# thu-nics/Rad-NeRF

Measured on AMD Instinct MI355X. Metric: million samples/s fwd+bwd, 8192 rays, model_zoo_size=2; rgb L∞ vs ref, higher is better.
Workload: dtype f16/f32

## Files before the change

### include/radnerf.h

```cpp
#ifndef RADNERF_H
#define RADNERF_H

#include <stdint.h>

#ifdef __cplusplus
extern "C" {
#endif

#define RN_ABI_VERSION 9
#define RN_FX_STATS_BYTES 640
int rn_version(void);
const char* rn_last_error(void);
const char* rn_abi_signatures(void);
void rn_set_debug_flags(int flags);
int rn_debug_cycles(unsigned long long* out);
int rn_set_level_pairing(uint64_t pairing);

int rn_ray_aabb_intersect(const float* rays_o, const float* rays_d, const float* centers,
                          const float* half_sizes, int64_t n_rays, int64_t n_voxels,
                          int32_t max_hits, int32_t* hit_cnt, float* hits_t,
                          int64_t* hits_voxel_idx, void* stream);

int rn_ray_sphere_intersect(const float* rays_o, const float* rays_d, const float* centers,
                            const float* radii, int64_t n_rays, int64_t n_spheres,
// ... 182 lines not shown
int rn_igrad_to_f32(int64_t n, int32_t* igrad_lo, int32_t* igrad_carry, const float* scale,
                    float* grid_grad, void* stream);

int rn_field_fwd_merged(const float* ts, const int32_t* ray_of, const float* rays_o,
                        const float* rays_d, const int32_t* seg_base, const int32_t* seg_count,
                        const int32_t* chunk_desc, int32_t* queue,
                        int64_t n_rays, int32_t n_models, const void* grid_f16,
                        const uint32_t* level_offset, const uint32_t* level_hsize,
                        const uint32_t* level_res, const float* level_scale,
                        const float* xyz_min, const float* extent, const void* frags,
                        float* sigma, float* rgb, void* feat_cache, const int32_t* mstart,
                        const int32_t* perm, int32_t blocks, int32_t threads, void* stream);

int rn_field_fwd_levels(const float* ts, const int32_t* ray_of, const float* rays_o,
                        const float* rays_d, const int32_t* seg_base, const int32_t* seg_count,
                        int64_t n_rays, int32_t n_models, const void* grid_f16,
                        const uint32_t* level_offset, const uint32_t* level_hsize,
                        const uint32_t* level_res, const float* level_scale,
                        const float* xyz_min, const float* extent, const void* frags,
                        float* sigma, float* rgb, void* feat_cache, const int32_t* mstart,
                        const int32_t* perm, uint32_t* planes, int64_t plane_stride, void* prep,
                        int32_t prep_ready, int32_t enc_blocks, int32_t mlp_blocks, int32_t* xq,
                        void* stream);

int rn_gate_fwd(const float* in0, const float* in1, int32_t stride, int64_t n_rays,
                int32_t n_models, const void* frags, float* gate, float* importance,
                int32_t n_blocks, void* stream);
int rn_gate_bwd(const float* in0, const float* in1, int32_t stride, int64_t n_rays,
                int32_t n_models, const void* frags, const float* dL_dgate, float* dw,
                int32_t n_params, const void* dinput_frags, float* dL_dinput,
                int32_t n_blocks, void* stream);

int rn_field_dinput(const float* xyzs, const float* dirs, int64_t n_samples, const float* ts,
                    const int32_t* ray_of, const float* rays_o, const float* rays_d,
                    const int32_t* seg_base, const int32_t* seg_count, int32_t n_models,
                    const void* grid_f16, const uint32_t* level_offset,
                    const uint32_t* level_hsize, const uint32_t* level_res,
                    const float* level_scale, const float* xyz_min, const float* extent,
                    const void* frags, const void* dinput_frags, const float* dL_dsigma,
                    const float* dL_drgb, const void* feat_cache, float* dL_dxyz,
                    float* dL_ddir, int32_t blocks_per_model, void* stream);
int rn_density_update_sampled(const void* grid_ptrs, const void* bitfield_ptrs, int32_t n_models,
                              int32_t cascades, int32_t grid_size, float scale,
                              float density_threshold, float decay, uint64_t seed,
                              const void* grid_f16, const uint32_t* level_offset,
                              const uint32_t* level_hsize, const uint32_t* level_res,
// ... 90 lines not shown
```

### rad-nerf_amd/csrc/field.hip

```cpp
#include "rn_field.h"
#include "rn_bin.h"
#pragma clang fp contract(off)

static int g_field_dbg = 0;
static uint64_t g_level_pairing = 0;
__device__ unsigned long long g_rn_cyc[8];

namespace {

template <int MODE, int CACHE>
__global__ void __launch_bounds__(256, FWD_MIN_WAVES)
k_field_fwd(FieldArgs a) {
    __shared__ __attribute__((aligned(16))) rn_half sW[FIELD_FWD_FRAGS * RN_FRAG_HALFS];
    __shared__ LvTab sT;
    const int k = blockIdx.y;
    rn_block_copy16(sW, a.frags + (size_t)k * FIELD_FRAGS * RN_FRAG_HALFS,
                    FIELD_FWD_FRAGS * RN_FRAG_BYTES);
    lv_stage(sT, a.gm);
    __syncthreads();
    int64_t base, n;
    sample_range(a, MODE, k, base, n);
    const int64_t n_tiles = (n + 31) / 32;
    const int waves = blockDim.x / RN_WAVE;
    const int lane = rn_lane(), h = lane >> 5;
    for (int64_t tile = (int64_t)blockIdx.x * waves + threadIdx.x / RN_WAVE; tile < n_tiles;
         tile += (int64_t)gridDim.x * waves) {
        rn_lds_order();
        FwdState st;
// ... 1123 lines not shown
    }
    lv_stage(sT, a.gm);
    const int waves = blockDim.x / RN_WAVE;
    const int wid = __builtin_amdgcn_readfirstlane(threadIdx.x / RN_WAVE);
    const int lane = rn_lane(), c = lane & 31, h = lane >> 5;
    int ticket = 0, n_chunks = 0;
    if (threadIdx.x == 0) { n_chunks = m.queue[1]; ticket = atomicAdd(m.queue + 2, 1); }

    auto mlp_tile = [&](const int32_t* ch, int u) {
        const int k = u % K, t = u / K;
        const int n_k = ch[2 + FM_KMAX + k];
        if (t * 32 >= n_k) return;
        rn_lds_order();
        const int i = t * 32 + c;
        const bool valid = i < n_k;
        const int64_t s = ch[2 + k] + (valid ? i : 0);
        FwdState st;
        float ux, uy, uz;
        constexpr int TC = ENC_M ? CACHE_READ_NT : CACHE;
        const rn_half* W = GW ? a.frags + (size_t)k * FIELD_FRAGS * RN_FRAG_HALFS
                              : sWm + (size_t)k * FIELD_FWD_FRAGS * RN_FRAG_HALFS;
        tile_forward_s<1, TC>(a, sT, W, s, valid, TC != CACHE_NONE ? cache_slot(a, s) : nullptr,
                              st, ux, uy, uz);
        if (valid && h == 0) {
            a.sigma[s] = expf(st.g0);
            a.rgb[3 * s + 0] = sigmoidf(st.out[0]);
            a.rgb[3 * s + 1] = sigmoidf(st.out[1]);
            a.rgb[3 * s + 2] = sigmoidf(st.out[2]);
        }
    };
    auto mlp_tiles = [&](const int32_t* ch) {
        int max_t = 0;
        for (int k = 0; k < K; ++k) max_t = max(max_t, (ch[2 + FM_KMAX + k] + 31) >> 5);
        return max_t * K;
    };

    bool prev_live = false;
    for (int it = 0;; ++it) {
        int32_t* cur = sCh[it & 1];
        const int32_t* prev = sCh[(it & 1) ^ 1];
        __syncthreads();
        if (threadIdx.x == 0) {
            const int ch = ticket;
            ticket = atomicAdd(m.queue + 2, 1);
            int4 d[CH_DESC / 4];
            if (ch < n_chunks) {
#pragma unroll
                for (int q = 0; q < CH_DESC / 4; ++q)
                    d[q] = reinterpret_cast<const int4*>(m.desc + (size_t)ch * CH_DESC)[q];
            }
            const int32_t* di = reinterpret_cast<const int32_t*>(d);
            cur[0] = ch < n_chunks ? di[0] : B;
// ... 14 lines not shown
        if (!live && !prev_live) break;
        int p_base = 0, n_p = 0;
        if (live) { p_base = m.mstart[cur[0]]; n_p = m.mstart[cur[1]] - p_base; }
        const int nA = (n_p + 31) >> 5;
        const int nB = prev_live ? mlp_tiles(prev) : 0;
        for (int u = wid; u < nA + nB; u += waves) {
            if (u >= nA) { mlp_tile(prev, u - nA); continue; }
            const int q = u * 32 + c;
            const bool valid = q < n_p;
            const int64_t s = m.perm[p_base + (valid ? q : 0)];
            float x, y, z, dx, dy, dz;
            load_sample<1>(a, s, x, y, z, dx, dy, dz);
            const float ux = unit_coord(x, a.xyz_min[0], a.extent[0]);
            const float uy = unit_coord(y, a.xyz_min[1], a.extent[1]);
            const float uz = unit_coord(z, a.xyz_min[2], a.extent[2]);
            half8 e0, e1;
            encode_lane(a, sT, rn_rsrc(a.grid, a.grid_bytes), h, ux, uy, uz, valid, e0, e1);
            if (valid) { half8* fc = cache_slot(a, s); fc[0] = e0; fc[1] = e1; }
        }
        prev_live = live;
    }
}


__global__ void __launch_bounds__(256)
k_enc_prep(FieldArgs a, MergeArgs m, float4* __restrict__ prep) {
    const int P = m.mstart[m.n_rays];
    for (int p = blockIdx.x * blockDim.x + threadIdx.x; p < P; p += gridDim.x * blockDim.x) {
        const int s = m.perm[p];
        float x, y, z, dx, dy, dz;
        load_sample<1>(a, s, x, y, z, dx, dy, dz);
        prep[p] = make_float4(unit_coord(x, a.xyz_min[0], a.extent[0]),
                              unit_coord(y, a.xyz_min[1], a.extent[1]),
                              unit_coord(z, a.xyz_min[2], a.extent[2]), __int_as_float(s));
    }
}

__global__ void __launch_bounds__(256)
k_field_encode_levels(FieldArgs a, MergeArgs m, const float4* __restrict__ prep,
                      int32_t* __restrict__ xq, uint64_t pairing) {
    __shared__ LvTab sT;
    lv_stage(sT, a.gm);
    __syncthreads();
    const int g = blockIdx.x & 7;
    if (xq && threadIdx.x == 0) {
        uint32_t xcc;
// ... 61 lines not shown
    for (int kb = k_lo; kb <= k_hi; kb += FM_LDS_K) {
        const int ke = min(k_hi, kb + FM_LDS_K - 1);
        __syncthreads();
        for (int k = kb; k <= ke; ++k)
            rn_block_copy16(sWm + (size_t)(k - kb) * FIELD_FWD_FRAGS * RN_FRAG_HALFS,
                            a.frags + (size_t)k * FIELD_FRAGS * RN_FRAG_HALFS,
                            FIELD_FWD_FRAGS * RN_FRAG_BYTES);
        __syncthreads();
        const int ua = max(u0, first[kb]), ub = min(u1, first[ke + 1]);
        for (int u = ua + wid; u < ub; u += waves) {
            int k = kb;
            while (k < ke && u >= first[k + 1]) ++k;
            const int t = u - first[k];
            const int n_k = sSeg[1][k];
            const int i = t * 32 + c;
            const bool valid = i < n_k;
            const int64_t s = sSeg[0][k] + (valid ? i : 0);
            FwdState st;
            float ux, uy, uz;
            rn_lds_order();
            tile_forward_s<1, CACHE_PLANES>(a, sT, sWm + (size_t)(k - kb) * FIELD_FWD_FRAGS * RN_FRAG_HALFS,
                                            s, valid, a.feat ? cache_slot(a, s) : nullptr, st,
                                            ux, uy, uz);
            if (valid && h == 0) {
                a.sigma[s] = expf(st.g0);
                a.rgb[3 * s + 0] = sigmoidf(st.out[0]);
                a.rgb[3 * s + 1] = sigmoidf(st.out[1]);
                a.rgb[3 * s + 2] = sigmoidf(st.out[2]);
            }
        }
    }
}


__global__ void __launch_bounds__(256)
k_seed_max(const int32_t* __restrict__ seg_base, const int32_t* __restrict__ seg_count,
           const float* __restrict__ sigma, const float* __restrict__ dsigma,
           const float* __restrict__ drgb, uint32_t* __restrict__ mbits) {
    const int k = blockIdx.y;
    const int64_t base = seg_base[k], n = seg_count[k];
    float mx = 0.f;
    for (int64_t i = (int64_t)blockIdx.x * blockDim.x + threadIdx.x; i < n;
         i += (int64_t)gridDim.x * blockDim.x) {
        const int64_t s = base + i;
        mx = fmaxf(mx, fabsf(dsigma[s] * sigma[s]));
        mx = fmaxf(mx, fmaxf(fabsf(drgb[3 * s]), fmaxf(fabsf(drgb[3 * s + 1]), fabsf(drgb[3 * s + 2]))));
    }
    mx = rn_wave_max(mx);
    if (rn_lane() == 0 && mx > 0.f && isfinite(mx)) atomicMax(mbits, __float_as_uint(mx));
}

__global__ void k_seed_scale(const uint32_t* __restrict__ mbits, float* __restrict__ scale) {
// ... 788 lines not shown
            RN_CHECK_LAUNCH();
            return 0;
        }
    }
    if (fx_mode == 5) {
        k_field_bwd_merged<CACHE_READ, false, 5><<<blocks, blk, 0, st>>>(a, m, G, F);
    } else if (fx_mode == 4) {
        k_field_bwd_merged<CACHE_READ, false, 4><<<blocks, blk, 0, st>>>(a, m, G, F);
    } else if (fx_mode == 2) {
        k_field_bwd_merged<CACHE_READ, false, 2><<<blocks, blk, 0, st>>>(a, m, G, F);
    } else if (fx_mode == 3) {
        k_field_bwd_merged<CACHE_READ, false, 3><<<blocks, blk, 0, st>>>(a, m, G, F);
    } else if (igrad_lo) {
        if (feat_cache) k_field_bwd_merged<CACHE_READ, false, 1><<<blocks, blk, 0, st>>>(a, m, G, F);
        else k_field_bwd_merged<CACHE_NONE, false, 1><<<blocks, blk, 0, st>>>(a, m, G, F);
    } else {
        if (feat_cache) k_field_bwd_merged<CACHE_READ, false, 0><<<blocks, blk, 0, st>>>(a, m, G, F);
        else k_field_bwd_merged<CACHE_NONE, false, 0><<<blocks, blk, 0, st>>>(a, m, G, F);
    }
    RN_CHECK_LAUNCH();
    return 0;
}

int rn_field_fwd_merged(const float* ts, const int32_t* ray_of, const float* rays_o,
                        const float* rays_d, const int32_t* seg_base, const int32_t* seg_count,
                        const int32_t* chunk_desc, int32_t* queue,
                        int64_t n_rays, int32_t n_models, const void* grid_f16,
                        const uint32_t* level_offset, const uint32_t* level_hsize,
                        const uint32_t* level_res, const float* level_scale,
                        const float* xyz_min, const float* extent, const void* frags,
                        float* sigma, float* rgb, void* feat_cache, const int32_t* mstart,
                        const int32_t* perm, int32_t blocks, int32_t threads, void* stream) {
    RN_CHECK_ARG(n_rays >= 1 && n_models >= 1 && n_models <= FM_KMAX && blocks >= 1,
                 "bad sizes (n_models <= 8)");
    RN_CHECK_ARG(threads >= 64 && threads <= 1024 && threads % 64 == 0, "threads: 64..1024, waves");
    RN_CHECK_ARG(ts && ray_of && rays_o && rays_d && seg_base && seg_count &&
                 chunk_desc && queue && grid_f16 && level_offset && level_hsize && level_res &&
                 level_scale && xyz_min && extent && frags && sigma && rgb, "null pointer");
    RN_CHECK_ARG(!(mstart || perm) || (mstart && perm && feat_cache),
                 "merged-order encoding needs mstart, perm and the encoding cache");
    FieldArgs a{};
    fill_args(a, xyz_min, extent, level_offset, level_hsize, level_res, level_scale);
    a.dbg = rn_dbg(g_field_dbg);
    a.grid = (const rn_half*)grid_f16; a.frags = (const rn_half*)frags;
    a.sigma = sigma; a.rgb = rgb; a.feat = (rn_half*)feat_cache;
    a.ts = ts; a.ray_of = ray_of; a.rays_o = rays_o; a.rays_d = rays_d;
    a.seg_base = seg_base; a.seg_count = seg_count;
    MergeArgs m{};
    m.desc = chunk_desc; m.queue = queue;
    m.mstart = mstart; m.perm = perm;
    m.n_rays = (int)n_rays; m.n_models = n_models;
    const bool gw = n_models > FM_LDS_K;
    const size_t lds = gw ? 0 : (size_t)n_models * FIELD_FWD_FRAGS * RN_FRAG_BYTES;
    hipStream_t st = (hipStream_t)stream;
    if (hipMemsetAsync(queue + 2, 0, sizeof(int32_t), st) != hipSuccess) {
        rn_set_error("%s: ticket reset failed", __func__);
        return 2;
    }
#define RN_FM_LAUNCH(C, E)                                                                     \
    do {                                                                                       \
        if (gw) k_field_fwd_merged<C, E, true><<<blocks, threads, 0, st>>>(a, m);              \
        else k_field_fwd_merged<C, E, false><<<blocks, threads, lds, st>>>(a, m);              \
    } while (0)
    if (mstart) RN_FM_LAUNCH(CACHE_WRITE, true);
    else if (feat_cache) RN_FM_LAUNCH(CACHE_WRITE, false);
    else RN_FM_LAUNCH(CACHE_NONE, false);
#undef RN_FM_LAUNCH
    RN_CHECK_LAUNCH();
    return 0;
}

int rn_field_fwd_levels(const float* ts, const int32_t* ray_of, const float* rays_o,
                        const float* rays_d, const int32_t* seg_base, const int32_t* seg_count,
                        int64_t n_rays, int32_t n_models, const void* grid_f16,
                        const uint32_t* level_offset, const uint32_t* level_hsize,
                        const uint32_t* level_res, const float* level_scale,
                        const float* xyz_min, const float* extent, const void* frags,
                        float* sigma, float* rgb, void* feat_cache, const int32_t* mstart,
                        const int32_t* perm, uint32_t* planes, int64_t plane_stride, void* prep,
                        int32_t prep_ready, int32_t enc_blocks, int32_t mlp_blocks, int32_t* xq,
                        void* stream) {
    RN_CHECK_ARG(n_rays >= 1 && n_models >= 1 && n_models <= FM_KMAX && plane_stride >= 1,
                 "bad sizes (n_models <= 8)");
    RN_CHECK_ARG(enc_blocks >= 8 && enc_blocks % 8 == 0 && mlp_blocks >= 1,
                 "bad launch (enc_blocks: a multiple of 8)");
    RN_CHECK_ARG(ts && ray_of && rays_o && rays_d && seg_base && seg_count && grid_f16 &&
                 level_offset && level_hsize && level_res && level_scale && xyz_min && extent &&
                 frags && sigma && rgb && mstart && perm && planes && prep, "null pointer");
    FieldArgs a{};
    fill_args(a, xyz_min, extent, level_offset, level_hsize, level_res, level_scale);
    a.dbg = rn_dbg(g_field_dbg);
    a.grid = (const rn_half*)grid_f16; a.frags = (const rn_half*)frags;
    a.sigma = sigma; a.rgb = rgb; a.feat = (rn_half*)feat_cache;
    a.planes = planes; a.plane_stride = plane_stride;
    a.ts = ts; a.ray_of = ray_of; a.rays_o = rays_o; a.rays_d = rays_d;
    a.seg_base = seg_base; a.seg_count = seg_count;
    MergeArgs m{};
    m.mstart = mstart; m.perm = perm; m.n_rays = (int)n_rays; m.n_models = n_models;
    hipStream_t st = (hipStream_t)stream;
    if (xq && (hipMemsetAsync(xq, 0, 64 * sizeof(int32_t), st) != hipSuccess ||
               hipMemsetAsync(xq + 64, 0xff, 16 * sizeof(int32_t), st) != hipSuccess ||
               hipMemsetAsync(xq + 80, 0, 16 * sizeof(int32_t), st) != hipSuccess)) {
        rn_set_error("%s: probe reset failed", __func__);
        return 2;
    }
    if (!prep_ready) k_enc_prep<<<1024, 256, 0, st>>>(a, m, (float4*)prep);
    uint64_t pairing = g_level_pairing;
    if (pairing == 0)
        for (int g = 0; g < 8; ++g) pairing |= (uint64_t)(g | ((RN_L - 1 - g) << 4)) << (8 * g);
    k_field_encode_levels<<<enc_blocks, 256, 0, st>>>(a, m, (const float4*)prep, xq, pairing);
    k_field_mlp_planes<<<mlp_blocks, 1024,
                         (size_t)min(n_models, FM_LDS_K) * FIELD_FWD_FRAGS * RN_FRAG_BYTES, st>>>(
        a, n_models);
    RN_CHECK_LAUNCH();
    return 0;
}

int rn_seed_scale(const int32_t* seg_base, const int32_t* seg_count, int32_t n_models,
                  const float* sigma, const float* dL_dsigma, const float* dL_drgb,
// ... 76 lines not shown
```

### rad-nerf_amd/csrc/render.hip

```cpp
#include "rn_field.h"
#include "rn_march.h"
#pragma clang fp contract(off)

namespace {

#define RT_WAVES 4
#ifndef RT_MIN_BLOCKS
#define RT_MIN_BLOCKS 1
#endif

struct TileSink {
    float* ts; float* dts;
    __device__ __forceinline__ void emit(int s, float, float, float, float t, float dt) const {
        ts[s] = t; dts[s] = dt;
    }
};

struct RenderArgs {
    const float* hits;
    const uint8_t* bitfields;
    int64_t bitfield_bytes;
    MarchCfg mc;
    float* opacity; float* depth; float* rgb;
    int32_t* n_samples;
// ... 2 lines not shown

__device__ __forceinline__ float rd_lane(float v, int l) {
    return __int_as_float(__builtin_amdgcn_readlane(__float_as_int(v), l));
}

__global__ void __launch_bounds__(RT_WAVES * 64, RT_MIN_BLOCKS)
k_render_test(FieldArgs a, RenderArgs g) {
    __shared__ __attribute__((aligned(16))) rn_half sW[FIELD_FWD_FRAGS * RN_FRAG_HALFS];
    __shared__ LvTab sT;
    __shared__ float sTs[RT_WAVES][32], sDt[RT_WAVES][32];
    const int k = blockIdx.y;
    rn_block_copy16(sW, a.frags + (size_t)k * FIELD_FRAGS * RN_FRAG_HALFS,
                    FIELD_FWD_FRAGS * RN_FRAG_BYTES);
    lv_stage(sT, a.gm);
    __syncthreads();
    const int wid = threadIdx.x / RN_WAVE, lane = rn_lane(), c = lane & 31;
    const uint8_t* bits = g.bitfields + (size_t)k * g.bitfield_bytes;
    const TileSink sink{sTs[wid], sDt[wid]};
    const int wave0 = __builtin_amdgcn_readfirstlane(blockIdx.x * RT_WAVES + wid);
    const int n_waves = gridDim.x * RT_WAVES;
    for (int r = wave0; r < g.n_rays; r += n_waves) {
        const float ox = a.rays_o[3 * r], oy = a.rays_o[3 * r + 1], oz = a.rays_o[3 * r + 2];
        const float dx = a.rays_d[3 * r], dy = a.rays_d[3 * r + 1], dz = a.rays_d[3 * r + 2];
        float t = g.hits[2 * r];
        const float t2 = g.hits[2 * r + 1];
        float co = 0.f, cr = 0.f, cg = 0.f, cb = 0.f, cd = 0.f;
        int n_tot = 0, tiles = 0;
        for (;;) {
            if (++tiles > g.max_samples) { n_tot = -1; break; }
            const int cap = min(32, g.max_samples - n_tot);
            const int n = __builtin_amdgcn_readfirstlane(march_ray_wave<true, TileSink, true>(
                ox, oy, oz, dx, dy, dz, t, t2, cap, 0, bits, g.mc, sink));
            n_tot += n;
            if (n == 0) break;
            __builtin_amdgcn_fence(__ATOMIC_SEQ_CST, "wavefront");
            const bool valid = c < n;
            const float tc = valid ? sTs[wid][c] : 0.f, dtc = valid ? sDt[wid][c] : 0.f;
            t = sTs[wid][n - 1] + sDt[wid][n - 1];
            const float x = fmaf(tc, dx, ox), y = fmaf(tc, dy, oy), z = fmaf(tc, dz, oz);
            FwdState st;
            float ux, uy, uz;
            tile_forward_pos<CACHE_NONE>(a, sT, sW, x, y, z, dx, dy, dz, valid, nullptr, st,
                                         ux, uy, uz);
            const float sig = expf(st.g0);
            const float r0 = sigmoidf(st.out[0]), r1 = sigmoidf(st.out[1]), r2 = sigmoidf(st.out[2]);
            float T = 1.0f - co;
            bool stop = false;
            for (int s = 0; s < n; ++s) {
                const float ts_ = rd_lane(tc, s), dl = rd_lane(dtc, s);
                const float al = 1.0f - rn_exp_det(-rd_lane(sig, s) * dl);
                const float w = al * T;
                cr = fmaf(w, rd_lane(r0, s), cr);
                cg = fmaf(w, rd_lane(r1, s), cg);
                cb = fmaf(w, rd_lane(r2, s), cb);
                cd = fmaf(w, ts_, cd);
                co += w;
                T *= 1.0f - al;
                if (T <= g.thr) { stop = true; break; }
            }
            if (stop || n < cap || n_tot >= g.max_samples) break;
            __builtin_amdgcn_fence(__ATOMIC_SEQ_CST, "wavefront");
        }
        if (lane == 0) {
            const size_t o = (size_t)k * g.n_rays + r;
            g.opacity[o] = co; g.depth[o] = cd;
            g.rgb[3 * o] = cr; g.rgb[3 * o + 1] = cg; g.rgb[3 * o + 2] = cb;
// ... 42 lines not shown
```

### rad-nerf_amd/csrc/rn_field.h

```cpp
#pragma once
#include "rn_mlp.h"
#pragma clang fp contract(off)

#define RN_L 16
#define FIELD_FWD_FRAGS 24
#define FIELD_FRAGS 46
#define FIELD_PARAMS 9472
#define FIELD_DW_TILES 12
#ifndef FWD_MIN_WAVES
#define FWD_MIN_WAVES 2
#endif

struct GridMeta {
    uint32_t offset[RN_L];
    uint32_t hsize[RN_L];
    uint32_t res[RN_L];
    float scale[RN_L];
    uint32_t dense_mask;
    uint32_t pow2_mask;
};

struct FieldArgs {
    const float* xyzs; const float* dirs;
    const float* ts; const int32_t* ray_of; const float* rays_o; const float* rays_d;
    const int32_t* seg_base; const int32_t* seg_count;
    int64_t n_fixed;
    const rn_half* grid;
    float* grid_grad;
    const rn_half* frags;
    float* dw;
    float* sigma; float* rgb;
    const float* dsigma; const float* drgb;
    rn_half* feat;
    const uint32_t* planes;
    int64_t plane_stride;
    float xyz_min[3]; float extent[3];
    uint32_t grid_bytes;
    int dbg;
    GridMeta gm;
};

namespace {


__device__ __forceinline__ void sample_range(const FieldArgs& a, int MODE, int k, int64_t& base,
                                             int64_t& n) {
    if (MODE == 0) { base = 0; n = a.n_fixed; }
    else { base = a.seg_base[k]; n = a.seg_count[k]; }
}

template <int MODE>
__device__ __forceinline__ void load_sample(const FieldArgs& a, int64_t s, float& x, float& y,
                                            float& z, float& dx, float& dy, float& dz) {
    if (MODE == 0) {
        x = a.xyzs[3 * s]; y = a.xyzs[3 * s + 1]; z = a.xyzs[3 * s + 2];
        dx = a.dirs[3 * s]; dy = a.dirs[3 * s + 1]; dz = a.dirs[3 * s + 2];
    } else {
        const int r = (rn_dbg(a.dbg) & 8192) ? 0 : a.ray_of[s];
        const float t = a.ts[s];
        dx = a.rays_d[3 * r]; dy = a.rays_d[3 * r + 1]; dz = a.rays_d[3 * r + 2];
        x = fmaf(t, dx, a.rays_o[3 * r]);
        y = fmaf(t, dy, a.rays_o[3 * r + 1]);
        z = fmaf(t, dz, a.rays_o[3 * r + 2]);
    }
}

__device__ __forceinline__ float unit_coord(float v, float mn, float ext) {
    return fminf(fmaxf((v - mn) / ext, 0.0f), 1.0f);
}

__device__ __forceinline__ int lane_level(int q, int h) { return 2 * h + (q & 1) + 4 * (q >> 1); }

struct LvTab {
    uint32_t off[RN_L];
    uint32_t hs[RN_L];
    uint32_t res[RN_L];
    uint32_t res2[RN_L];
    float sc[RN_L];
};

__device__ __forceinline__ void lv_stage(LvTab& t, const GridMeta& gm) {
    const int i = threadIdx.x;
    if (i < RN_L) {
        t.off[i] = gm.offset[i]; t.hs[i] = gm.hsize[i]; t.res[i] = gm.res[i]; t.sc[i] = gm.scale[i];
        t.res2[i] = gm.res[i] * gm.res[i];
    }
}
// ... 286 lines not shown
    a0 = rn_mfma(rn_frag(W, 8), st.sh, a0); a0 = rn_mfma(rn_frag(W, 9), st.gin, a0);
    a1 = rn_mfma(rn_frag(W, 10), st.sh, a1); a1 = rn_mfma(rn_frag(W, 11), st.gin, a1);
    rn_acc_to_frags<true>(a0, st.r1[0], st.r1[1]);
    rn_acc_to_frags<true>(a1, st.r1[2], st.r1[3]);
    a0 = rn_zero16(); a1 = rn_zero16();
#pragma unroll
    for (int q = 0; q < 4; ++q) {
        a0 = rn_mfma(rn_frag(W, 12 + q), st.r1[q], a0);
        a1 = rn_mfma(rn_frag(W, 16 + q), st.r1[q], a1);
    }
    rn_acc_to_frags<true>(a0, st.r2[0], st.r2[1]);
    rn_acc_to_frags<true>(a1, st.r2[2], st.r2[3]);
    st.out = rn_zero16();
#pragma unroll
    for (int q = 0; q < 4; ++q) st.out = rn_mfma(rn_frag(W, 20 + q), st.r2[q], st.out);
}

__device__ __forceinline__ float sigmoidf(float x) { return 1.0f / (1.0f + expf(-x)); }

enum { CACHE_NONE = 0, CACHE_WRITE = 1, CACHE_READ = 2,
       CACHE_READ_NT = 3,
       CACHE_PLANES = 4 };

template <int CACHE>
__device__ __forceinline__ void tile_forward_pos(const FieldArgs& a, const LvTab& T, const rn_half* W,
                                                 float x, float y, float z, float dx, float dy,
                                                 float dz, bool valid, half8* fc, FwdState& st,
                                                 float& ux, float& uy, float& uz);

template <int MODE, int CACHE>
__device__ __forceinline__ void tile_forward_s(const FieldArgs& a, const LvTab& T, const rn_half* W,
                                               int64_t s, bool valid, half8* fc, FwdState& st,
                                               float& ux, float& uy, float& uz) {
    float x = 0.f, y = 0.f, z = 0.f, dx = 1.f, dy = 0.f, dz = 0.f;
    if (CACHE == CACHE_PLANES) {
        const int h = rn_lane() >> 5;
        typedef uint32_t u4v __attribute__((ext_vector_type(4)));
        u4v w0 = {0u, 0u, 0u, 0u}, w1 = {0u, 0u, 0u, 0u};
        if (valid) {
            const uint32_t* pl = a.planes + s;
#pragma unroll
            for (int q = 0; q < 4; ++q) {
                w0[q] = pl[(size_t)lane_level(q, h) * a.plane_stride];
                w1[q] = pl[(size_t)lane_level(q + 4, h) * a.plane_stride];
            }
        }
        st.e0 = __builtin_bit_cast(half8, w0); st.e1 = __builtin_bit_cast(half8, w1);
    }
    if (valid) load_sample<MODE>(a, s, x, y, z, dx, dy, dz);
    tile_forward_pos<CACHE>(a, T, W, x, y, z, dx, dy, dz, valid, fc, st, ux, uy, uz);
}

template <int CACHE>
__device__ __forceinline__ void tile_forward_rays(const FieldArgs& a, const LvTab& T,
                                                  const rn_half* W, int64_t s, bool valid,
                                                  half8* fc, const float* sRays, int r0, int nr,
                                                  FwdState& st, float& ux, float& uy, float& uz) {
    float x = 0.f, y = 0.f, z = 0.f, dx = 1.f, dy = 0.f, dz = 0.f;
    if (valid) {
        const int r = a.ray_of[s];
        const float t = a.ts[s];
        const uint32_t q = (uint32_t)(r - r0);
        float ox, oy, oz;
        if (q < (uint32_t)nr) {
            typedef __attribute__((address_space(3))) const float lds_f;
            lds_f* p = (lds_f*)sRays + 6 * q;
            ox = p[0]; oy = p[1]; oz = p[2]; dx = p[3]; dy = p[4]; dz = p[5];
        } else {
            ox = a.rays_o[3 * r]; oy = a.rays_o[3 * r + 1]; oz = a.rays_o[3 * r + 2];
            dx = a.rays_d[3 * r]; dy = a.rays_d[3 * r + 1]; dz = a.rays_d[3 * r + 2];
        }
        x = fmaf(t, dx, ox);
        y = fmaf(t, dy, oy);
        z = fmaf(t, dz, oz);
    }
    tile_forward_pos<CACHE>(a, T, W, x, y, z, dx, dy, dz, valid, fc, st, ux, uy, uz);
}

template <int CACHE>
__device__ __forceinline__ void tile_forward_pos(const FieldArgs& a, const LvTab& T, const rn_half* W,
                                                 float x, float y, float z, float dx, float dy,
                                                 float dz, bool valid, half8* fc, FwdState& st,
                                                 float& ux, float& uy, float& uz) {
    const int h = rn_lane() >> 5;
    ux = unit_coord(x, a.xyz_min[0], a.extent[0]);
    uy = unit_coord(y, a.xyz_min[1], a.extent[1]);
    uz = unit_coord(z, a.xyz_min[2], a.extent[2]);
    if (CACHE == CACHE_PLANES) {
        if (valid && fc) { fc[0] = st.e0; fc[1] = st.e1; }
    } else if (CACHE == CACHE_READ || CACHE == CACHE_READ_NT) {
        st.e0 = rn_zero8(); st.e1 = rn_zero8();
        if (valid && CACHE == CACHE_READ) { st.e0 = fc[0]; st.e1 = fc[1]; }
        if (valid && CACHE == CACHE_READ_NT) {
            st.e0 = __builtin_nontemporal_load(fc);
            st.e1 = __builtin_nontemporal_load(fc + 1);
        }
    } else {
        if (rn_dbg(a.dbg) & 256) { st.e0 = rn_zero8(); st.e1 = rn_zero8(); asm volatile("" :: "v"(ux), "v"(uy), "v"(uz)); }
        else encode_lane(a, T, rn_rsrc(a.grid, a.grid_bytes), h, ux, uy, uz, valid, st.e0, st.e1);
        if (CACHE == CACHE_WRITE && valid) { fc[0] = st.e0; fc[1] = st.e1; }
    }
    st.sh = sh_lane(dx, dy, dz, h);
    if (rn_dbg(a.dbg) & 4096) {
        st.out = rn_zero16(); st.g0 = 0.f;
        asm volatile("" :: "v"(st.e0), "v"(st.e1), "v"(st.sh));
    } else {
        mlp_forward(W, st);
    }
}

__device__ __forceinline__ half8* cache_slot(const FieldArgs& a, int64_t s) {
    return reinterpret_cast<half8*>(a.feat) + ((s >> 5) * 64 + (s & 31) + 32 * (rn_lane() >> 5)) * 2;
}

template <int MODE, int CACHE>
__device__ __forceinline__ void tile_forward(const FieldArgs& a, const LvTab& T, const rn_half* W,
                                             int64_t base, int64_t n, int64_t tile, FwdState& st,
                                             bool& valid, int64_t& s, float& ux, float& uy,
                                             float& uz) {
    const int lane = rn_lane(), c = lane & 31;
    const int64_t i = tile * 32 + c;
    valid = i < n;
    s = base + (valid ? i : 0);
    half8* fc = CACHE == CACHE_NONE ? nullptr
              : reinterpret_cast<half8*>(a.feat) + (((base >> 5) + tile) * 64 + lane) * 2;
// ... 21 lines not shown
```

### rad-nerf_amd/radnerf_amd/_lib.py

```python
import ctypes
import os

_HERE = os.path.dirname(os.path.abspath(__file__))
LIB_PATH = os.environ.get("RADNERF_LIB", os.path.join(_HERE, "librn.so"))
ABLATION_LIB_PATH = os.environ.get("RADNERF_ABL_LIB", os.path.join(_HERE, "librn_abl.so"))

P = ctypes.c_void_p
I32 = ctypes.c_int32
I64 = ctypes.c_int64
F32 = ctypes.c_float
F64 = ctypes.c_double
U64 = ctypes.c_uint64

SIGNATURES = {
    "rn_ray_aabb_intersect": [P, P, P, P, I64, I64, I32, P, P, P, P],
    "rn_ray_sphere_intersect": [P, P, P, P, I64, I64, I32, P, P, P, P],
    "rn_raymarching_train_bw": [P, P, P, P, I64, P, P, P],
    "rn_ml_march_bw": [P, P, I64, I32, P, P, P, P, P, P],
    "rn_field_dinput": [P, P, I64, P, P, P, P, P, P, I32, P, P, P, P, P, P, P, P, P, P, P, P, P,
                        P, I32, P],
    "rn_field_density": [P, I64, P, P, P, P, P, P, P, P, P, P, P],
    "rn_debug_cycles": [P],
    "rn_set_level_pairing": [ctypes.c_uint64],
    "rn_density_update_sampled": [P, P, I32, I32, I32, F32, F32, F32, U64, P, P, P, P, P, P, P,
# ... 28 lines not shown
    "rn_bwd_plan": [P, P, P, P, P, I64, I32, I32, I32, I32, I32, I32, I32, P, P, P, P, P,
                    P, P, P, P, P, P],
    "rn_field_bwd_merged": [P, P, P, P, P, P, P, P, P, P, I64, I32, I32, P, P, P, P, P, P,
                            P, P, P, P, P, P, P, P, I64, P, I32, I32, P, P, P, P, P, P,
                            P, I32, P, P, P, I32, P],
    "rn_grid_fx_fold": [P, P, P, P, P, P, P, P, P, P],
    "rn_grid_bin_layout": [P],
    "rn_debug_gb_cycles": [P],
    "rn_grid_slice_bits": [P, P],
    "rn_grid_record_encode": [P, I64, P],
    "rn_grid_record_decode": [P, I64, P],
    "rn_grid_bin": [P, P, P, P, P, P, P, I32, I32, P],
    "rn_grid_sum": [P, P, P, P, P, P, I32, P, P, P, I32, I32, P],
    "rn_grid_bin_check": [P, P, P, P, P, P, P, I32, P, P, P, P, P],
    "rn_grid_binned_fold": [P, P, P, P, P, P, P, P, I32, P, P, P, P, P, P],
    "rn_render_test": [P, P, P, I64, I32, P, I64, I32, F32, F32, I32, I32, P, P, P, P, P, P, P,
                       P, F32, P, P, P, P, I32, P],
    "rn_seed_scale": [P, P, I32, P, P, P, P, P, P],
    "rn_igrad_to_f32": [I64, P, P, P, P, P],
    "rn_field_fwd_merged": [P, P, P, P, P, P, P, P, I64, I32, P, P, P, P, P, P, P, P, P, P, P,
                            P, P, I32, I32, P],
    "rn_field_fwd_levels": [P, P, P, P, P, P, I64, I32, P, P, P, P, P, P, P, P, P, P, P, P, P,
                            P, I64, P, I32, I32, I32, P, P],
    "rn_gate_fwd": [P, P, I32, I64, I32, P, P, P, I32, P],
    "rn_gate_bwd": [P, P, I32, I64, I32, P, P, P, I32, P, P, I32, P],
    "rn_nerf_loss": [P, P, P, P, P, P, I64, I32, F32, F32, F32, P, P, P, P, P, P],
    "rn_adam": [P, P, P, P, I64, F64, F64, F64, F64, I32, F32, P, I64, P],
    "rn_get_rays": [P, P, P, P, I64, P, P, P, P, P],
    "rn_get_rays_pose": [P, P, P, P, P, P, I64, P, P, P, P, P],
    "rn_get_rays_pose_bw": [P, P, P, P, P, I64, I64, P, P, P, P, P, P, P],
    "rn_sample_batch": [P, I32, I64, I64, P, P, P, P, P, U64, I64, I32, I64, I32, P, P, P, P, P,
                        P, P, P, P],
    "rn_ml_combine_test": [P, P, P, P, P, I64, I32, I64, P, P, P, P, P],
    "rn_image_sse": [P, P, I64, P, P, P],
    "rn_ssim": [P, P, I32, I32, I32, P, P, P, P],
    "rn_minmax_finite": [P, I64, I64, P, P, P],
    "rn_quantize_u8": [P, I64, P, P],
    "rn_colormap_u8": [P, I64, I64, P, P, I32, P, P],
    "rn_gate_map_u8": [P, I64, I32, P, I32, P, P],
    "rn_pack_f16": [P, I64, P, I64, I32, I64, P, P],
    "rn_to_f16": [P, I64, P, P],
    "rn_morton3d": [P, I64, P, P],
    "rn_morton3d_invert": [P, I64, P, P],
    "rn_packbits": [P, I64, F32, P, P],
    "rn_scatter_max": [P, P, I64, P, P],
    "rn_mark_invisible_cells": [P, I32, F32, F32, F32, F32, I32, I32, F32, P, P, I32, I32, I32,
# ... 109 lines not shown
```

### rad-nerf_amd/radnerf_amd/fused.py

```python
import collections

import torch

from . import layout as LY
from ._lib import lib

MAX_SAMPLES = 1024
NEAR_DISTANCE = 0.01
SEG_ALIGN = 128
FX_STATS_BYTES = 640


GB_SUM_FAULT = 18
GB_CTL_READ = GB_SUM_FAULT + 1


def clamp_split(split_level):
    return max(0, min(15, int(split_level)))


def _stream(dev):
    return torch.cuda.current_stream(dev).cuda_stream


# ... 11 lines not shown
        i = dict(device=device, dtype=torch.int32)
        self.counts = torch.empty(K, B, **i)
        self.offsets = torch.empty(K, B, **i)
        self.seg = torch.zeros(2 * K + 2, **i)
        self.used = torch.empty(K, B, **i)
        self.ts = torch.empty(cap, **f)
        self.deltas = torch.empty(cap, **f)
        self.ray_of = torch.empty(cap, **i)
        self.sigma = torch.empty(cap, **f)
        self.rgb = torch.empty(cap, 3, **f)
        self.ws = torch.empty(cap, **f)
        self.dsigma = torch.empty(cap, **f)
        self.drgb = torch.empty(cap, 3, **f)
        self.opacity_k = torch.empty(K, B, **f)
        self.depth_k = torch.empty(K, B, **f)
        self.rgb_k = torch.empty(K, B, 3, **f)
        self.dgate = torch.empty(B, K, **f)
        self.stage_ts = torch.empty(K * B * max_samples, **f)
        self.stage_dt = torch.empty(K * B * max_samples, **f)
        self.feat = torch.empty((cap + 31) // 32 * 32, 32, device=device, dtype=torch.float16)
        self.mstart = torch.empty(B + 1, **i)
        self.perm = torch.empty(cap, **i)
        self.queue = torch.zeros(3, **i)
        self._bwd_scratch = None
        self._chunks = None
        self._dist_k = None
        self.generation = 0

    @property
    def dist_k(self):
        if self._dist_k is None:
            self._dist_k = torch.empty(self.K, self.B, device=self.device, dtype=torch.float32)
        return self._dist_k

    def chunk_list(self, max_chunk, min_chunk, head_chunks=0, balance_blocks=0):
        cap = (head_chunks + self.capacity // max_chunk + self.capacity // (8 * min_chunk) +
               max_chunk // min_chunk + 3 + balance_blocks)
        if self._chunks is None or self._chunks.numel() < cap + 1:
            self._chunks = torch.empty(cap + 1, device=self.device, dtype=torch.int32)
            self._chunk_desc = torch.empty(cap + 1, 20, device=self.device, dtype=torch.int32)
        return cap, self._chunks

    def level_buffers(self, stream=None):
        rows = self.feat.shape[0]
        key = (str(self.device), int(stream) if stream is not None else 0)
        cur = _LEVEL_SCRATCH.get(key)
# ... 52 lines not shown

class FusedMLRenderer:

    def __init__(self, model, gating_net, n_rays, device=None, fwd_blocks=None, bwd_blocks=None,
                 capacity=None):
        self.model, self.gate = model, gating_net
        self.device = device or model.mlp_params.device
        self.ws = Workspace(n_rays, model.size, self.device, capacity=capacity)
        K = model.size
        bf = [getattr(model, f"density_bitfield_{i}") for i in range(K)]
        self.bitfield_bytes = bf[0].numel()
        self.fwd_blocks = fwd_blocks or max(1, 2048 // K)
        self.bwd_blocks = bwd_blocks or max(1, 256 // K)
        self.feat_cache = True
        self.merged_bwd = 1 <= model.size <= 8
        self.merged_fwd = 1 < model.size <= 8
        self.merged_encode = model.size > 1
        self.merged_fwd_blocks = 256
        self.merged_fwd_threads = 1024
        self.level_fwd = self.merged_bwd or self.merged_fwd
        self.plan_prep = True
        self.level_enc_blocks = 4096
        self.level_mlp_blocks = 256
        self.merged_blocks = 256
        rk = n_rays * model.size
        self.max_chunk = 256 if rk <= 1024 else (512 if rk <= 4096 else 1024)
        if model.size >= 8 and rk > 4096:
            self.max_chunk = 12288
        elif model.size >= 4 and rk > 4096 and float(model.scale) > 0.5:
            self.max_chunk = 4096
        elif model.size >= 2 and rk > 4096 and float(model.scale) <= 0.5:
            self.max_chunk = 1536
        self.int_grad = False
        self.grid_fx = rk > 1024
        self.grid_bin = self.grid_fx and float(model.scale) > 0.5
        self.bin_f32_levels = (9 if model.size >= 8 else 8) if self.grid_bin else 0
        if not self.grid_bin and model.xyz_encoder.params.numel() > (1 << 28):
            self.grid_fx = False
        self.bin_records_per_pair = 6912
        self.min_chunk = 512
        if float(model.scale) > 0.5:
            if model.size >= 8 and n_rays >= 8192:
                self.min_chunk = 1536
        self.fx_f32_levels = ()
        self.head_chunk = self.max_chunk if float(model.scale) <= 0.5 and rk > 1024 else 0
        self.balance_chunks = True
# ... 57 lines not shown

    def bitfields(self):
        K = self.model.size
        bf = [getattr(self.model, f"density_bitfield_{i}") for i in range(K)]
        if all(b.data_ptr() == bf[0].data_ptr() + i * self.bitfield_bytes for i, b in enumerate(bf)):
            return bf[0]
        self._bf = torch.stack(bf).contiguous()
        return self._bf

    def forward(self, rays_o, rays_d, gate_in2, noise, bg, T_threshold=1e-4,
                exp_step_factor=0.0, distortion=False):
        m, g, w, L = self.model, self.gate, self.ws, lib()
        B, K, G = rays_o.shape[0], m.size, g.out_dim
        assert B == w.B and noise.shape == (K, B)
        st = _stream(rays_o.device)
        out_gate = torch.empty(B, G, device=rays_o.device)
        imp = torch.zeros(G, device=rays_o.device)
        side = self._side(rays_o.device)
        main = torch.cuda.current_stream(rays_o.device)
        if G == 1:
            out_gate.fill_(1.0)
            imp.fill_(float(B))
            side.wait_stream(main)
        else:
            frags = g.packed_frags()
            side.wait_stream(main)
            self._ev("gate_fwd", L.gate_fwd, rays_o.data_ptr(), gate_in2.data_ptr(), 3, B, G,
                     frags.data_ptr(), out_gate.data_ptr(), imp.data_ptr(),
                     max(1, min(256, (B + 127) // 128)), side.cuda_stream, stream=side)
        bits = self.bitfields()
        march = (rays_o.data_ptr(), rays_d.data_ptr(), m.center.data_ptr(),
                 m.half_size.data_ptr(), NEAR_DISTANCE, noise.data_ptr(), bits.data_ptr(),
                 self.bitfield_bytes, K, m.cascades, float(m.scale), float(exp_step_factor),
                 m.grid_size, MAX_SAMPLES, B)
        self._ev("march", L.ml_march_count, *march, w.counts.data_ptr(),
                 w.stage_ts.data_ptr(), w.stage_dt.data_ptr(), st)
        self._ev("scan", L.scan_segments, w.counts.data_ptr(), K, B, SEG_ALIGN,
                 w.offsets.data_ptr(), w.seg_base.data_ptr(), w.seg_count.data_ptr(),
                 w.meta.data_ptr(), st)
        self._ev("compact", L.ml_compact, w.counts.data_ptr(), w.offsets.data_ptr(), B, K,
                 MAX_SAMPLES, w.stage_ts.data_ptr(), w.stage_dt.data_ptr(), w.ts.data_ptr(),
                 w.deltas.data_ptr(), w.ray_of.data_ptr(), st)
        if self.merged_bwd or self.merged_fwd:
            self._plan(st, rays_o, rays_d if self.level_fwd and self.plan_prep else None)
        self._field(True, rays_o, rays_d, st)
        comp = (w.sigma.data_ptr(), w.rgb.data_ptr(), w.deltas.data_ptr(),
                w.ts.data_ptr(), w.counts.data_ptr(), w.offsets.data_ptr(), B, K,
                float(T_threshold), w.used.data_ptr(), w.opacity_k.data_ptr(),
                w.depth_k.data_ptr(), w.rgb_k.data_ptr(), w.ws.data_ptr())
        self._dist_forward = bool(distortion)
        if distortion:
            self._ev("composite_dist_fw", L.ml_composite_dist_fw, *comp, w.dist_k.data_ptr(), st)
        else:
            self._ev("composite_fw", L.ml_composite_fw, *comp, st)
        ok, dk, rk = self._gather_model_outputs()
        rgb = torch.empty(B, 3, device=rays_o.device)
        opacity = torch.empty(B, device=rays_o.device)
        depth = torch.empty(B, G, device=rays_o.device)
        main.wait_stream(side)
        out_gate.record_stream(side)
        imp.record_stream(side)
        self._ev("combine_fw", L.ml_combine_fw, out_gate.data_ptr(), ok.data_ptr(), dk.data_ptr(),
                        rk.data_ptr(), bg.data_ptr(), B, G, rgb.data_ptr(),
                        opacity.data_ptr(), depth.data_ptr(), st)
        return rgb, opacity, depth, out_gate, imp

    def _gather_model_outputs(self):
        return self._model_outputs()

    def _model_outputs(self):
        w = self.ws
        return w.opacity_k, w.depth_k, w.rgb_k

    def _local_cols(self, x):
        return x

    def _plan(self, st, rays_o=None, rays_d=None):
        w, L, m = self.ws, lib(), self.model
        prep = w.level_buffers(st)[1] if rays_d is not None else None
        self._min_chunk = min(self.min_chunk, self.max_chunk)
        head_n = self.merged_blocks if self.head_chunk else 0
        head = min(self.head_chunk, self.max_chunk)
        bal = self.merged_blocks if self.balance_chunks else 0
        self._cap_chunks, self._chunks = w.chunk_list(self.max_chunk, self._min_chunk, head_n, bal)
        self._ev("bwd_plan", L.bwd_plan, w.counts.data_ptr(), w.offsets.data_ptr(),
                 w.seg_base.data_ptr(), w.seg_count.data_ptr(), w.ts.data_ptr(), w.B, w.K,
                 head_n, head, self.max_chunk, self._min_chunk, bal, self._cap_chunks,
                 w.mstart.data_ptr(), w.perm.data_ptr(), self._chunks.data_ptr(),
                 w._chunk_desc.data_ptr(), w.queue.data_ptr(),
                 None if prep is None else rays_o.data_ptr(),
                 None if prep is None else rays_d.data_ptr(),
                 None if prep is None else m._h_min.ctypes.data,
                 None if prep is None else m._h_ext.ctypes.data,
                 None if prep is None else prep.data_ptr(), st)
        self._plan_key = (self.max_chunk, self._min_chunk, head_n, head, bal)
        self._prep_ready = prep is not None

    def _field(self, fwd, rays_o, rays_d, st, grid_grad=None, dw=None):
        m, w, L = self.model, self.ws, lib()
        lo, lh, lr, ls = m.xyz_encoder.level_ptrs()
        common = (None, None, 0, w.ts.data_ptr(), w.ray_of.data_ptr(), rays_o.data_ptr(),
                  rays_d.data_ptr(), w.seg_base.data_ptr(), w.seg_count.data_ptr(), m.size,
                  m.xyz_encoder.params_f16().data_ptr(), lo, lh, lr, ls, m._h_min.ctypes.data,
                  m._h_ext.ctypes.data, m.packed_frags().data_ptr())
        if fwd and self.level_fwd and (self.merged_bwd or self.merged_fwd):
            planes, prep = w.level_buffers(st)
            self._ev("field_fwd", L.field_fwd_levels, w.ts.data_ptr(), w.ray_of.data_ptr(),
                     rays_o.data_ptr(), rays_d.data_ptr(), w.seg_base.data_ptr(),
                     w.seg_count.data_ptr(), w.B, m.size, *common[10:], w.sigma.data_ptr(),
                     w.rgb.data_ptr(), w.feat.data_ptr(), w.mstart.data_ptr(), w.perm.data_ptr(),
                     planes.data_ptr(), planes.shape[1], prep.data_ptr(),
                     int(getattr(self, "_prep_ready", False)), self.level_enc_blocks,
                     self.level_mlp_blocks, None, st)
            self._prep_ready = False
        elif fwd and self.merged_fwd:
            self._ev("field_fwd", L.field_fwd_merged, w.ts.data_ptr(), w.ray_of.data_ptr(),
                     rays_o.data_ptr(), rays_d.data_ptr(), w.seg_base.data_ptr(),
                     w.seg_count.data_ptr(), w._chunk_desc.data_ptr(),
                     w.queue.data_ptr(), w.B, m.size, *common[10:], w.sigma.data_ptr(),
                     w.rgb.data_ptr(), w.feat.data_ptr() if self.feat_cache else None,
                     *((w.mstart.data_ptr(), w.perm.data_ptr())
                       if self.feat_cache and self.merged_encode else (None, None)),
                     self.merged_fwd_blocks, self.merged_fwd_threads, st)
        elif fwd:
            self._ev("field_fwd", L.field_fwd, *common, w.sigma.data_ptr(), w.rgb.data_ptr(),
                     w.feat.data_ptr() if self.feat_cache else None, self.fwd_blocks, st)
        elif self.merged_bwd:
# ... 409 lines not shown
```

Before: 1196.

## Precompute per-ray SH direction encoding on side stream and split activation stores across half-waves

Adds a kernel that computes the spherical-harmonics direction encoding once per ray into a half8 table on the side stream. The merged and level forward field kernels then read it by ray index instead of recomputing SH for every sample. Output activation stores are also restructured so both half-waves each compute and write two of the four outputs, using a permlane swap. This trades per-sample SH arithmetic for an extra table read, a small extra kernel and cross-stream synchronisation, and it adds global binding state.

```diff
diff --git a/include/radnerf.h b/include/radnerf.h
--- a/include/radnerf.h
+++ b/include/radnerf.h
@@ -228,6 +228,9 @@
                         const int32_t* perm, uint32_t* planes, int64_t plane_stride, void* prep,
                         int32_t prep_ready, int32_t enc_blocks, int32_t mlp_blocks, int32_t* xq,
                         void* stream);
+
+int rn_dir_sh(const float* rays_d, int64_t n_rays, void* table, void* stream);
+int rn_bind_dir_sh(const void* table, int64_t n_rays);
 
 int rn_gate_fwd(const float* in0, const float* in1, int32_t stride, int64_t n_rays,
                 int32_t n_models, const void* frags, float* gate, float* importance,
diff --git a/rad-nerf_amd/csrc/field.hip b/rad-nerf_amd/csrc/field.hip
--- a/rad-nerf_amd/csrc/field.hip
+++ b/rad-nerf_amd/csrc/field.hip
@@ -4,6 +4,14 @@
 
 static int g_field_dbg = 0;
 static uint64_t g_level_pairing = 0;
+static thread_local const void* g_dir_sh = nullptr;
+static thread_local int64_t g_dir_sh_rays = 0;
+static const half8* dir_sh_take(int64_t& n_rays) {
+    const void* t = g_dir_sh;
+    n_rays = g_dir_sh_rays;
+    g_dir_sh = nullptr; g_dir_sh_rays = 0;
+    return (const half8*)t;
+}
 __device__ unsigned long long g_rn_cyc[8];
 
 namespace {
@@ -1173,12 +1181,7 @@
                               : sWm + (size_t)k * FIELD_FWD_FRAGS * RN_FRAG_HALFS;
         tile_forward_s<1, TC>(a, sT, W, s, valid, TC != CACHE_NONE ? cache_slot(a, s) : nullptr,
                               st, ux, uy, uz);
-        if (valid && h == 0) {
-            a.sigma[s] = expf(st.g0);
-            a.rgb[3 * s + 0] = sigmoidf(st.out[0]);
-            a.rgb[3 * s + 1] = sigmoidf(st.out[1]);
-            a.rgb[3 * s + 2] = sigmoidf(st.out[2]);
-        }
+        store_activations(a, st, s, valid, h);
     };
     auto mlp_tiles = [&](const int32_t* ch) {
         int max_t = 0;
@@ -1239,6 +1242,14 @@
     }
 }
 
+
+__global__ void __launch_bounds__(256)
+k_dir_sh(int n_rays, const float* __restrict__ rays_d, half8* __restrict__ table) {
+    const int i = blockIdx.x * blockDim.x + threadIdx.x;
+    if (i >= 2 * n_rays) return;
+    const int r = i >> 1;
+    table[i] = sh_lane(rays_d[3 * r], rays_d[3 * r + 1], rays_d[3 * r + 2], i & 1);
+}
 
 __global__ void __launch_bounds__(256)
 k_enc_prep(FieldArgs a, MergeArgs m, float4* __restrict__ prep) {
@@ -1346,12 +1357,7 @@
             tile_forward_s<1, CACHE_PLANES>(a, sT, sWm + (size_t)(k - kb) * FIELD_FWD_FRAGS * RN_FRAG_HALFS,
                                             s, valid, a.feat ? cache_slot(a, s) : nullptr, st,
                                             ux, uy, uz);
-            if (valid && h == 0) {
-                a.sigma[s] = expf(st.g0);
-                a.rgb[3 * s + 0] = sigmoidf(st.out[0]);
-                a.rgb[3 * s + 1] = sigmoidf(st.out[1]);
-                a.rgb[3 * s + 2] = sigmoidf(st.out[2]);
-            }
+            store_activations(a, st, s, valid, h);
         }
     }
 }
@@ -2186,6 +2192,24 @@
     return 0;
 }
 
+int rn_dir_sh(const float* rays_d, int64_t n_rays, void* table, void* stream) {
+    RN_CHECK_ARG(n_rays >= 1 && n_rays < (1ll << 30), "bad sizes");
+    RN_CHECK_ARG(rays_d && table, "null pointer");
+    RN_CHECK_ARG(((uintptr_t)table & 15u) == 0, "table must be 16-B aligned");
+    k_dir_sh<<<nblk(2 * n_rays, 256), 256, 0, (hipStream_t)stream>>>((int)n_rays, rays_d,
+                                                                      (half8*)table);
+    RN_CHECK_LAUNCH();
+    return 0;
+}
+
+int rn_bind_dir_sh(const void* table, int64_t n_rays) {
+    g_dir_sh = nullptr; g_dir_sh_rays = 0;
+    RN_CHECK_ARG(!table || (n_rays >= 1 && ((uintptr_t)table & 15u) == 0),
+                 "table: 16-B aligned, n_rays >= 1");
+    g_dir_sh = table; g_dir_sh_rays = table ? n_rays : 0;
+    return 0;
+}
+
 int rn_field_fwd_merged(const float* ts, const int32_t* ray_of, const float* rays_o,
                         const float* rays_d, const int32_t* seg_base, const int32_t* seg_count,
                         const int32_t* chunk_desc, int32_t* queue,
@@ -2195,6 +2219,9 @@
                         const float* xyz_min, const float* extent, const void* frags,
                         float* sigma, float* rgb, void* feat_cache, const int32_t* mstart,
                         const int32_t* perm, int32_t blocks, int32_t threads, void* stream) {
+    int64_t sh_rays = 0;
+    const half8* dir_sh = dir_sh_take(sh_rays);
+    RN_CHECK_ARG(!dir_sh || sh_rays == n_rays, "the bound SH table is for another ray count");
     RN_CHECK_ARG(n_rays >= 1 && n_models >= 1 && n_models <= FM_KMAX && blocks >= 1,
                  "bad sizes (n_models <= 8)");
     RN_CHECK_ARG(threads >= 64 && threads <= 1024 && threads % 64 == 0, "threads: 64..1024, waves");
@@ -2210,6 +2237,7 @@
     a.sigma = sigma; a.rgb = rgb; a.feat = (rn_half*)feat_cache;
     a.ts = ts; a.ray_of = ray_of; a.rays_o = rays_o; a.rays_d = rays_d;
     a.seg_base = seg_base; a.seg_count = seg_count;
+    a.dir_sh = dir_sh;
     MergeArgs m{};
     m.desc = chunk_desc; m.queue = queue;
     m.mstart = mstart; m.perm = perm;
@@ -2244,6 +2272,9 @@
                         const int32_t* perm, uint32_t* planes, int64_t plane_stride, void* prep,
                         int32_t prep_ready, int32_t enc_blocks, int32_t mlp_blocks, int32_t* xq,
                         void* stream) {
+    int64_t sh_rays = 0;
+    const half8* dir_sh = dir_sh_take(sh_rays);
+    RN_CHECK_ARG(!dir_sh || sh_rays == n_rays, "the bound SH table is for another ray count");
     RN_CHECK_ARG(n_rays >= 1 && n_models >= 1 && n_models <= FM_KMAX && plane_stride >= 1,
                  "bad sizes (n_models <= 8)");
     RN_CHECK_ARG(enc_blocks >= 8 && enc_blocks % 8 == 0 && mlp_blocks >= 1,
@@ -2259,6 +2290,7 @@
     a.planes = planes; a.plane_stride = plane_stride;
     a.ts = ts; a.ray_of = ray_of; a.rays_o = rays_o; a.rays_d = rays_d;
     a.seg_base = seg_base; a.seg_count = seg_count;
+    a.dir_sh = dir_sh;
     MergeArgs m{};
     m.mstart = mstart; m.perm = perm; m.n_rays = (int)n_rays; m.n_models = n_models;
     hipStream_t st = (hipStream_t)stream;
diff --git a/rad-nerf_amd/csrc/render.hip b/rad-nerf_amd/csrc/render.hip
--- a/rad-nerf_amd/csrc/render.hip
+++ b/rad-nerf_amd/csrc/render.hip
@@ -48,6 +48,7 @@
     for (int r = wave0; r < g.n_rays; r += n_waves) {
         const float ox = a.rays_o[3 * r], oy = a.rays_o[3 * r + 1], oz = a.rays_o[3 * r + 2];
         const float dx = a.rays_d[3 * r], dy = a.rays_d[3 * r + 1], dz = a.rays_d[3 * r + 2];
+        const half8 sh = sh_lane(dx, dy, dz, lane >> 5);
         float t = g.hits[2 * r];
         const float t2 = g.hits[2 * r + 1];
         float co = 0.f, cr = 0.f, cg = 0.f, cb = 0.f, cd = 0.f;
@@ -66,8 +67,7 @@
             const float x = fmaf(tc, dx, ox), y = fmaf(tc, dy, oy), z = fmaf(tc, dz, oz);
             FwdState st;
             float ux, uy, uz;
-            tile_forward_pos<CACHE_NONE>(a, sT, sW, x, y, z, dx, dy, dz, valid, nullptr, st,
-                                         ux, uy, uz);
+            tile_forward_pos<CACHE_NONE>(a, sT, sW, x, y, z, sh, valid, nullptr, st, ux, uy, uz);
             const float sig = expf(st.g0);
             const float r0 = sigmoidf(st.out[0]), r1 = sigmoidf(st.out[1]), r2 = sigmoidf(st.out[2]);
             float T = 1.0f - co;
diff --git a/rad-nerf_amd/csrc/rn_field.h b/rad-nerf_amd/csrc/rn_field.h
--- a/rad-nerf_amd/csrc/rn_field.h
+++ b/rad-nerf_amd/csrc/rn_field.h
@@ -34,6 +34,7 @@
     rn_half* feat;
     const uint32_t* planes;
     int64_t plane_stride;
+    const half8* dir_sh;
     float xyz_min[3]; float extent[3];
     uint32_t grid_bytes;
     int dbg;
@@ -51,18 +52,26 @@
 
 template <int MODE>
 __device__ __forceinline__ void load_sample(const FieldArgs& a, int64_t s, float& x, float& y,
-                                            float& z, float& dx, float& dy, float& dz) {
+                                            float& z, float& dx, float& dy, float& dz, int& r) {
     if (MODE == 0) {
+        r = 0;
         x = a.xyzs[3 * s]; y = a.xyzs[3 * s + 1]; z = a.xyzs[3 * s + 2];
         dx = a.dirs[3 * s]; dy = a.dirs[3 * s + 1]; dz = a.dirs[3 * s + 2];
     } else {
-        const int r = (rn_dbg(a.dbg) & 8192) ? 0 : a.ray_of[s];
+        r = (rn_dbg(a.dbg) & 8192) ? 0 : a.ray_of[s];
         const float t = a.ts[s];
         dx = a.rays_d[3 * r]; dy = a.rays_d[3 * r + 1]; dz = a.rays_d[3 * r + 2];
         x = fmaf(t, dx, a.rays_o[3 * r]);
         y = fmaf(t, dy, a.rays_o[3 * r + 1]);
         z = fmaf(t, dz, a.rays_o[3 * r + 2]);
     }
+}
+
+template <int MODE>
+__device__ __forceinline__ void load_sample(const FieldArgs& a, int64_t s, float& x, float& y,
+                                            float& z, float& dx, float& dy, float& dz) {
+    int r;
+    load_sample<MODE>(a, s, x, y, z, dx, dy, dz, r);
 }
 
 __device__ __forceinline__ float unit_coord(float v, float mn, float ext) {
@@ -395,11 +404,28 @@
        CACHE_READ_NT = 3,
        CACHE_PLANES = 4 };
 
+__device__ __forceinline__ void store_activations(const FieldArgs& a, const FwdState& st, int64_t s,
+                                                  bool valid, int h) {
+    auto from_lo = [](float v) {
+        const uint32_t u = __float_as_uint(v);
+        return __uint_as_float(__builtin_amdgcn_permlane32_swap(u, u, false, false)[0]);
+    };
+    const float o1 = from_lo(st.out[1]), o2 = from_lo(st.out[2]);
+    const float p0 = h ? o1 : st.g0;
+    const float p1 = h ? o2 : st.out[0];
+    const float e0 = expf(h ? -p0 : p0), e1 = expf(-p1);
+    const float v0 = h ? 1.0f / (1.0f + e0) : e0, v1 = 1.0f / (1.0f + e1);
+    if (valid) {
+        *(h ? a.rgb + 3 * s + 1 : a.sigma + s) = v0;
+        a.rgb[3 * s + (h ? 2 : 0)] = v1;
+    }
+}
+
 template <int CACHE>
 __device__ __forceinline__ void tile_forward_pos(const FieldArgs& a, const LvTab& T, const rn_half* W,
-                                                 float x, float y, float z, float dx, float dy,
-                                                 float dz, bool valid, half8* fc, FwdState& st,
-                                                 float& ux, float& uy, float& uz);
+                                                 float x, float y, float z, half8 sh, bool valid,
+                                                 half8* fc, FwdState& st, float& ux, float& uy,
+                                                 float& uz);
 
 template <int MODE, int CACHE>
 __device__ __forceinline__ void tile_forward_s(const FieldArgs& a, const LvTab& T, const rn_half* W,
@@ -420,8 +446,20 @@
         }
         st.e0 = __builtin_bit_cast(half8, w0); st.e1 = __builtin_bit_cast(half8, w1);
     }
-    if (valid) load_sample<MODE>(a, s, x, y, z, dx, dy, dz);
-    tile_forward_pos<CACHE>(a, T, W, x, y, z, dx, dy, dz, valid, fc, st, ux, uy, uz);
+    const int hl = rn_lane() >> 5;
+    half8 sh;
+    if (MODE == 1 && a.dir_sh) {
+        sh = rn_zero8();
+        if (valid) {
+            int r;
+            load_sample<MODE>(a, s, x, y, z, dx, dy, dz, r);
+            sh = a.dir_sh[2 * r + hl];
+        }
+    } else {
+        if (valid) load_sample<MODE>(a, s, x, y, z, dx, dy, dz);
+        sh = sh_lane(dx, dy, dz, hl);
+    }
+    tile_forward_pos<CACHE>(a, T, W, x, y, z, sh, valid, fc, st, ux, uy, uz);
 }
 
 template <int CACHE>
@@ -447,14 +485,15 @@
         y = fmaf(t, dy, oy);
         z = fmaf(t, dz, oz);
     }
-    tile_forward_pos<CACHE>(a, T, W, x, y, z, dx, dy, dz, valid, fc, st, ux, uy, uz);
+    tile_forward_pos<CACHE>(a, T, W, x, y, z, sh_lane(dx, dy, dz, rn_lane() >> 5), valid, fc, st,
+                            ux, uy, uz);
 }
 
 template <int CACHE>
 __device__ __forceinline__ void tile_forward_pos(const FieldArgs& a, const LvTab& T, const rn_half* W,
-                                                 float x, float y, float z, float dx, float dy,
-                                                 float dz, bool valid, half8* fc, FwdState& st,
-                                                 float& ux, float& uy, float& uz) {
+                                                 float x, float y, float z, half8 sh, bool valid,
+                                                 half8* fc, FwdState& st, float& ux, float& uy,
+                                                 float& uz) {
     const int h = rn_lane() >> 5;
     ux = unit_coord(x, a.xyz_min[0], a.extent[0]);
     uy = unit_coord(y, a.xyz_min[1], a.extent[1]);
@@ -473,7 +512,7 @@
         else encode_lane(a, T, rn_rsrc(a.grid, a.grid_bytes), h, ux, uy, uz, valid, st.e0, st.e1);
         if (CACHE == CACHE_WRITE && valid) { fc[0] = st.e0; fc[1] = st.e1; }
     }
-    st.sh = sh_lane(dx, dy, dz, h);
+    st.sh = sh;
     if (rn_dbg(a.dbg) & 4096) {
         st.out = rn_zero16(); st.g0 = 0.f;
         asm volatile("" :: "v"(st.e0), "v"(st.e1), "v"(st.sh));
diff --git a/rad-nerf_amd/radnerf_amd/_lib.py b/rad-nerf_amd/radnerf_amd/_lib.py
--- a/rad-nerf_amd/radnerf_amd/_lib.py
+++ b/rad-nerf_amd/radnerf_amd/_lib.py
@@ -74,6 +74,8 @@
                             P, P, I32, I32, P],
     "rn_field_fwd_levels": [P, P, P, P, P, P, I64, I32, P, P, P, P, P, P, P, P, P, P, P, P, P,
                             P, I64, P, I32, I32, I32, P, P],
+    "rn_dir_sh": [P, I64, P, P],
+    "rn_bind_dir_sh": [P, I64],
     "rn_gate_fwd": [P, P, I32, I64, I32, P, P, P, I32, P],
     "rn_gate_bwd": [P, P, I32, I64, I32, P, P, P, I32, P, P, I32, P],
     "rn_nerf_loss": [P, P, P, P, P, P, I64, I32, F32, F32, F32, P, P, P, P, P, P],
diff --git a/rad-nerf_amd/radnerf_amd/fused.py b/rad-nerf_amd/radnerf_amd/fused.py
--- a/rad-nerf_amd/radnerf_amd/fused.py
+++ b/rad-nerf_amd/radnerf_amd/fused.py
@@ -57,6 +57,7 @@
         self.mstart = torch.empty(B + 1, **i)
         self.perm = torch.empty(cap, **i)
         self.queue = torch.zeros(3, **i)
+        self.dir_sh = torch.empty(B, 2, 8, device=device, dtype=torch.float16)
         self._bwd_scratch = None
         self._chunks = None
         self._dist_k = None
@@ -155,6 +156,7 @@
         self.plan_prep = True
         self.level_enc_blocks = 4096
         self.level_mlp_blocks = 256
+        self.dir_sh = True
         self.merged_blocks = 256
         rk = n_rays * model.size
         self.max_chunk = 256 if rk <= 1024 else (512 if rk <= 4096 else 1024)
@@ -258,9 +260,11 @@
             out_gate.fill_(1.0)
             imp.fill_(float(B))
             side.wait_stream(main)
+            self._fill_dir_sh(rays_d, side)
         else:
             frags = g.packed_frags()
             side.wait_stream(main)
+            self._fill_dir_sh(rays_d, side)
             self._ev("gate_fwd", L.gate_fwd, rays_o.data_ptr(), gate_in2.data_ptr(), 3, B, G,
                      frags.data_ptr(), out_gate.data_ptr(), imp.data_ptr(),
                      max(1, min(256, (B + 127) // 128)), side.cuda_stream, stream=side)
@@ -279,6 +283,8 @@
                  w.deltas.data_ptr(), w.ray_of.data_ptr(), st)
         if self.merged_bwd or self.merged_fwd:
             self._plan(st, rays_o, rays_d if self.level_fwd and self.plan_prep else None)
+        if self._dir_sh_filled:
+            main.wait_event(self._dir_sh_event)
         self._field(True, rays_o, rays_d, st)
         comp = (w.sigma.data_ptr(), w.rgb.data_ptr(), w.deltas.data_ptr(),
                 w.ts.data_ptr(), w.counts.data_ptr(), w.offsets.data_ptr(), B, K,
@@ -301,6 +307,20 @@
                         opacity.data_ptr(), depth.data_ptr(), st)
         return rgb, opacity, depth, out_gate, imp
 
+    def _merged_or_level_fwd(self):
+        return bool(self.merged_fwd or (self.level_fwd and self.merged_bwd))
+
+    def _fill_dir_sh(self, rays_d, side):
+        self._dir_sh_filled = bool(self.dir_sh) and self._merged_or_level_fwd()
+        if not self._dir_sh_filled:
+            return
+        w = self.ws
+        self._ev("dir_sh", lib().dir_sh, rays_d.data_ptr(), w.B, w.dir_sh.data_ptr(),
+                 side.cuda_stream, stream=side)
+        if getattr(self, "_dir_sh_event", None) is None:
+            self._dir_sh_event = torch.cuda.Event()
+        self._dir_sh_event.record(side)
+
     def _gather_model_outputs(self):
         return self._model_outputs()
 
@@ -339,6 +359,9 @@
                   rays_d.data_ptr(), w.seg_base.data_ptr(), w.seg_count.data_ptr(), m.size,
                   m.xyz_encoder.params_f16().data_ptr(), lo, lh, lr, ls, m._h_min.ctypes.data,
                   m._h_ext.ctypes.data, m.packed_frags().data_ptr())
+        if fwd and getattr(self, "_dir_sh_filled", False) and self._merged_or_level_fwd():
+            L.bind_dir_sh(w.dir_sh.data_ptr(), w.B)
+            self._dir_sh_filled = False
         if fwd and self.level_fwd and (self.merged_bwd or self.merged_fwd):
             planes, prep = w.level_buffers(st)
             self._ev("field_fwd", L.field_fwd_levels, w.ts.data_ptr(), w.ray_of.data_ptr(),
```

New measurement: 1199 (median of 6 runs). Within noise of the previous version (+0.3%).
